# NVIDIA/audio-flamingo

Hardware: AMD Instinct MI355X
Metric: audio-sec/s + decoder tokens/s, AF3-7B bf16 train (higher is better)
Workload: dtype bf16; 1 GPU; AF3 (AF-Whisper 32L + Qwen2.5-7B 28L, MLP projector) bf16 train step fwd+bwd+AdamW, 30 s clips, S=1024; micro_batch_per_gpu=8, global_batch=8, seq_len=1024, parallelism=dp1, activation_checkpointing=False

## Files before the change

audio-flamingo_amd/csrc/gemm.hip:

```cpp
#include "gemm_common.h"
#include <vector>
#include <mutex>

namespace {

constexpr int BM = 128, BN = 128, BK = 64;
constexpr int ROWB = BK * 2;
constexpr int STAGE_BYTES = (BM + BN) * ROWB;
constexpr int NSTAGE = 2;

__global__ __launch_bounds__(256, 2) void gemm_nt_bf16_k128(GemmArgs p) {
    extern __shared__ __attribute__((aligned(16))) char smem[];
    const int tid = threadIdx.x;
    const int lane = tid & 63;
    const int wave = __builtin_amdgcn_readfirstlane(tid >> 6);
    const int wm = wave >> 1, wn = wave & 1;
    const int hi = lane >> 5, l31 = lane & 31;

    int tm, tn;
    gemm_tile_of_block(p, tm, tn);
    const int m0 = tm * BM, n0 = tn * BN;

    const bf16* a_src[4];
    const bf16* b_src[4];
// ... 140 lines not shown

__global__ __launch_bounds__(256) void gemm_splitk_reduce_kernel(GemmArgs p) {
    const int n4 = p.N >> 2;
    const int64_t total = (int64_t)p.M * n4;
    for (int64_t t = (int64_t)blockIdx.x * blockDim.x + threadIdx.x; t < total; t += (int64_t)gridDim.x * blockDim.x) {
        const int m = (int)(t / n4), n = (int)(t % n4) * 4;
        const float* src = p.ws + (int64_t)m * p.N + n;
        f32x4 acc = *(const f32x4*)src;
        for (int sp = 1; sp < p.splits; ++sp) {
            const f32x4 x = *(const f32x4*)(src + (int64_t)sp * p.M * p.N);
#pragma unroll
            for (int e = 0; e < 4; ++e) acc[e] += x[e];
        }
        float v[4] = {acc[0], acc[1], acc[2], acc[3]};
        gemm_epilogue_store4(p, m, n, v);
    }
}

struct ProfState {
    std::mutex mu;
    bool on = false;
    std::vector<hipEvent_t> pool;
    size_t used = 0;
    double flops = 0.0;
    int64_t launches = 0;
    struct Rec { int M, N, K, variant; };
    std::vector<Rec> recs;
};
ProfState g_prof;
int g_variant = 0;
[[maybe_unused]] int g_256_impl = 2;
int g_gm = 0;
int g_wide = 1;
int g_mfma = 0;

constexpr int mfma_shapes(int form) { return form == 0 ? AFK_MFMA_SHAPES_NT : form == 1 ? AFK_MFMA_SHAPES_NN : AFK_MFMA_SHAPES_TN; }
constexpr int AFK_MFMA_RULE_NT = 16, AFK_MFMA_RULE_NN = 32, AFK_MFMA_RULE_TN = 32;
int gemm_mfma_of(int form) {
    static const int env = [] {
        const char* e = getenv("AFK_GEMM_MFMA");
        return (e && e[0] >= '0' && e[0] <= '2' && !e[1]) ? e[0] - '0' : 0;
    }();
    const int sel = g_mfma ? g_mfma : env;
    if (sel == 1) return 32;
    if (sel == 2) return 16;
    return form == 0 ? AFK_MFMA_RULE_NT : form == 1 ? AFK_MFMA_RULE_NN : AFK_MFMA_RULE_TN;
}

hipEvent_t prof_next_event() {
    if (g_prof.used == g_prof.pool.size()) {
        hipEvent_t e;
        hipEventCreate(&e);
        g_prof.pool.push_back(e);
    }
    return g_prof.pool[g_prof.used++];
}

}

extern "C" int afk_gemm_set_variant(int v) {
    const int gm = (v >> 8) & 255, base = v & 15;
#ifdef AFK_PROBES
    AFK_REQUIRE(base >= 0 && base <= 14, "afk_gemm_set_variant: 14 = persistent tile loop with the next tile's prologue issued ahead of the epilogue stores (round-4 probe), 13 = 256x256 ping-pong as a persistent tile loop, 0 auto, 1 = 128x128, 2 = 256x256 8-wave ping-pong, 3 = 256x256 4-wave (4, 5: its timing probes), 6 = 256x256 8-wave free-running BK=64 (7, 8, 9: probes), 10 = 8-wave free-running BK=32 ring-10 (11: probe)");
#else
    AFK_REQUIRE(base >= 0 && base <= 2, "afk_gemm_set_variant: variant %d is a probe / rejected schedule; this libafk.so was built without -DAFK_PROBES (make PROBES=1)", base);
    AFK_REQUIRE((gm & 0xc0) == 0, "afk_gemm_set_variant: gm bits 6 / 7 are timing probes (wrong results); this libafk.so was built without -DAFK_PROBES");
#endif
    g_gm = gm;
    g_wide = (v & 16) ? 0 : 1;
    g_variant = base;
    return AFK_OK;
}

extern "C" int afk_gemm_set_mfma(int v) {
    AFK_REQUIRE(v >= 0 && v <= 2, "afk_gemm_set_mfma: %d (0 = dispatch rule, 1 = 32x32x16, 2 = 16x16x32)", v);
    constexpr int any = AFK_MFMA_SHAPES_NT | AFK_MFMA_SHAPES_NN | AFK_MFMA_SHAPES_TN;
    AFK_REQUIRE(v == 0 || (any >> (v - 1)) & 1, "afk_gemm_set_mfma: no 256x256 kernel of this libafk.so carries the %s shape; build with make PROBES=1",
                v == 1 ? "32x32x16" : "16x16x32");
    g_mfma = v;
    return AFK_OK;
}
extern "C" int afk_gemm_mfma_shapes(int form) { return form >= 0 && form <= 2 ? mfma_shapes(form) : 0; }

extern "C" int afk_prof_enable(int on) {
    std::lock_guard<std::mutex> lk(g_prof.mu);
    g_prof.on = on != 0;
    return AFK_OK;
}

extern "C" int afk_prof_reset(void) {
    std::lock_guard<std::mutex> lk(g_prof.mu);
    g_prof.used = 0;
    g_prof.flops = 0.0;
    g_prof.launches = 0;
    g_prof.recs.clear();
    return AFK_OK;
}

extern "C" int afk_prof_collect(double* total_ms, double* total_flops, int64_t* launches) {
    std::lock_guard<std::mutex> lk(g_prof.mu);
    double ms = 0.0;
// ... 26 lines not shown
    AFK_REQUIRE(M > 0 && N > 0 && K > 0, "afk_gemm_nt_bf16: bad shape %d %d %d", M, N, K);
    AFK_REQUIRE(!trans_a || trans_b, "afk_gemm_bf16: A^T with k-contiguous B is not implemented (NT, NN, TN are)");
    AFK_REQUIRE(trans_a || K % BK == 0, "afk_gemm_nt_bf16: K=%d must be a multiple of %d (pad the operand)", K, BK);
    AFK_REQUIRE(!trans_b || (N % 8 == 0 && N >= 8), "afk_gemm_bf16: N=%d must be a multiple of 8 for a reduction-major B", N);
    AFK_REQUIRE(!trans_a || (M % 8 == 0 && M >= 8), "afk_gemm_bf16: M=%d must be a multiple of 8 for a reduction-major A", M);
    AFK_REQUIRE(N % 4 == 0, "afk_gemm_nt_bf16: N=%d must be a multiple of 4", N);
    AFK_REQUIRE(lda % 8 == 0 && ldb % 8 == 0 && ldc % 4 == 0, "afk_gemm_nt_bf16: leading dims must keep 16-B (A,B) / 8-B (C) alignment");
    AFK_REQUIRE(!(flags & AFK_GEMM_BIAS) || bias, "afk_gemm_nt_bf16: BIAS flag without bias");
    AFK_REQUIRE(!(flags & AFK_GEMM_RESIDUAL) || (residual && ldr % 4 == 0), "afk_gemm_nt_bf16: RESIDUAL flag without residual");
    AFK_REQUIRE(!(flags & AFK_GEMM_SWIGLU_FWD) || (flags == AFK_GEMM_SWIGLU_FWD && !trans_a && !trans_b && preact_out && N % 256 == 0 && splits == 1 &&
                                                     ldc % 8 == 0 && (uintptr_t)C % 16 == 0 && (uintptr_t)preact_out % 16 == 0),
                "afk_gemm_nt_bf16: SWIGLU_FWD needs the NT form, preact_out, N = 2I with I %% 128 == 0 and no other flag");
    AFK_REQUIRE(!(flags & AFK_GEMM_SWIGLU_BWD) || (residual && ldr % 4 == 0 && ldc >= 2 * (int64_t)N && flags == AFK_GEMM_SWIGLU_BWD && splits == 1),
                "afk_gemm: SWIGLU_BWD needs the gate|up tensor as `residual`, a [M, 2N] output and no other epilogue flag");
    AFK_REQUIRE(((uintptr_t)A % 16 == 0) && ((uintptr_t)B % 16 == 0) && ((uintptr_t)C % 8 == 0), "afk_gemm_nt_bf16: misaligned pointer");
    GemmArgs p;
    p.A = (const bf16*)A;
    p.B = (const bf16*)B;
    p.C = C;
    p.C2 = preact_out;
    p.bias = (const bf16*)bias;
    p.R = (const bf16*)residual;
    p.lda = lda;
    p.ldb = ldb;
    p.ldc = ldc;
    p.ldr = ldr;
    p.M = M;
    p.N = N;
    p.K = K;
    p.flags = flags;
    p.res_mod = res_mod;
    p.alpha = alpha;
    p.gm = g_gm;
    p.splits = splits;
    p.ws = (float*)workspace;
    p.rope_cos = rope ? (const bf16*)rope->cos_t : nullptr;
    p.rope_sin = rope ? (const bf16*)rope->sin_t : nullptr;
    p.rope_pos = rope ? rope->pos : nullptr;
    p.rope_S = rope ? rope->S : 1;
    p.rope_cols = rope ? rope->cols : 0;
    const bool lanes_ok = rope && rope->cos_lanes && rope->sin_lanes && !rope->pos && rope->S % 32 == 0;
    p.rope_cos_lanes = lanes_ok ? (const bf16*)rope->cos_lanes : nullptr;
    p.rope_sin_lanes = lanes_ok ? (const bf16*)rope->sin_lanes : nullptr;
    {
        const bool f32 = (flags & AFK_GEMM_OUT_F32) != 0;
        bool w = N % 8 == 0 && ldc % 8 == 0 && (uintptr_t)C % (f32 ? 32 : 16) == 0;
        if (flags & AFK_GEMM_BIAS) w = w && (uintptr_t)bias % 16 == 0;
        if (flags & (AFK_GEMM_RESIDUAL | AFK_GEMM_SWIGLU_BWD)) w = w && ldr % 8 == 0 && (uintptr_t)residual % 16 == 0;
        if (preact_out) w = w && (uintptr_t)preact_out % 16 == 0;
        p.wide = w && g_wide ? 1 : 0;
    }
    const int64_t tiles256 = afk_cdiv(M, 256) * afk_cdiv(N, 256);
    const bool use256 = !gemv && (trans_b || (flags & AFK_GEMM_SWIGLU_FWD) || (splits == 1 && (g_variant >= 2 || (g_variant == 0 && tiles256 >= 192))));
    if (rope && (!use256 || !p.wide || trans_a || trans_b || splits != 1))
        return afk_set_error(AFK_ERR_UNSUPPORTED, "afk_gemm_nt_bf16_rope: needs the 256 x 256 NT kernel (>= 192 tiles) in its 16-byte epilogue form; use "
                                                  "afk_gemm_nt_bf16 + afk_rope_inplace for this shape");
#ifdef AFK_PROBES
    static const int env_impl = [] {
        const char* e = getenv("AFK_GEMM256");
        return (e && e[0] == 'p' && e[1] == 'e') ? 13 : (e && e[0] == 'p') ? 2 : (e && e[0] == 'w') ? 3 : (e && e[0] == 'f') ? 10 : 0;
    }();
    const int impl256 = (flags & (AFK_GEMM_SWIGLU_FWD | AFK_GEMM_ROPE)) ? 2 : g_variant >= 2 ? g_variant : (env_impl ? env_impl : g_256_impl);
    const bool w4 = use256 && !trans_b && impl256 >= 3 && impl256 <= 9;
    const bool f8 = use256 && !trans_b && impl256 >= 10 && impl256 <= 12;
    const bool persist = use256 && !trans_b && impl256 == 13;
    const bool persist_q = use256 && !trans_b && impl256 == 14;
// ... 130 lines not shown
```

audio-flamingo_amd/csrc/gemm256.hip:

```cpp
#include "gemm_common.h"

namespace {

constexpr int BM = 256, BN = 256, BK = 64;
constexpr int ROWB = 128;
constexpr int OP_BYTES = 256 * ROWB;
constexpr int BUF_BYTES = 2 * OP_BYTES;
constexpr int LDS_BYTES = 2 * BUF_BYTES;

#define AFK_VMCNT(n) asm volatile("s_waitcnt vmcnt(" #n ")" ::: "memory")
#define AFK_LGKMCNT0() asm volatile("s_waitcnt lgkmcnt(0)" ::: "memory")
#define AFK_BARRIER()                         \
    do {                                      \
        __builtin_amdgcn_sched_barrier(0);    \
        __builtin_amdgcn_s_barrier();         \
        __builtin_amdgcn_sched_barrier(0);    \
    } while (0)

template <int EPI, int MF>
__global__ __launch_bounds__(512, 1) void gemm_nt_bf16_k256(GemmArgs p) {
    extern __shared__ __attribute__((aligned(16))) char smem[];
    const int tid = threadIdx.x;
    const int lane = tid & 63;
    const int wave = __builtin_amdgcn_readfirstlane(tid >> 6);
    const int wm = wave >> 2, wn = wave & 3;
    const int hi = lane >> 5, l31 = lane & 31;

    int tm, tn;
    gemm_tile_of_block(p, tm, tn);
    const int m0 = tm * BM, n0 = tn * BN;

    const bf16* xsrc[6];
    int xdst[6];
    const bf16* ysrc[2];
    int ydst[2];
    {
        const int lrow = lane >> 3, pos = lane & 7;
#pragma unroll
        for (int j = 0; j < 6; ++j) {
            const int i = wave + 8 * j;
            const bool isB = i < 32;
            const int unit = isB ? i : ((i - 32) < 8 ? (i - 32) : (i - 32) + 8);
            const int rl = unit * 8 + lrow;
            const int chunk = pos ^ ((rl >> 1) & 7);
            if (isB) {
                const int r = (EPI == AFK_GEMM_SWIGLU_FWD) ? (rl < 128 ? tn * 128 + rl : (p.N >> 1) + tn * 128 + rl - 128) : min(n0 + rl, p.N - 1);
                xsrc[j] = p.B + (int64_t)r * p.ldb + chunk * 8;
            } else {
                const int r = min(m0 + rl, p.M - 1);
                xsrc[j] = p.A + (int64_t)r * p.lda + chunk * 8;
            }
            xdst[j] = (isB ? OP_BYTES : 0) + unit * 1024;
// ... 45 lines not shown
    AFK_BARRIER();
    if (wm == 1) AFK_BARRIER();

    bf16x8 bf[2][4], af[2][4];
    auto mfma_group = [&](auto acc0_, auto g_) {
        constexpr int ACC0 = decltype(acc0_)::value, g = decltype(g_)::value;
        if constexpr (MF == 32) {
#pragma unroll
            for (int i = 0; i < 2; ++i)
#pragma unroll
                for (int j = 0; j < 2; ++j) acc.mma(ACC0 + i, j, bf[j][g], af[i][g]);
        } else {
            constexpr int s = g >> 1, i = g & 1;
#pragma unroll
            for (int ih = 0; ih < 2; ++ih)
#pragma unroll
                for (int jt = 0; jt < 4; ++jt) acc.mma(2 * (ACC0 + i) + ih, jt, bf[jt >> 1][2 * (jt & 1) + s], af[i][2 * ih + s]);
        }
    };
    auto mfma_slot = [&](auto acc0_, auto q_) {
        constexpr int ACC0 = decltype(acc0_)::value, q = decltype(q_)::value;
        if constexpr (MF == 32) {
            constexpr int s = q >> 1, i = q & 1;
            acc.mma(ACC0 + i, 0, bf[0][s], af[i][s]);
            acc.mma(ACC0 + i, 1, bf[1][s], af[i][s]);
        } else {
            constexpr int s = q >> 2, i = (q >> 1) & 1, ih = q & 1;
#pragma unroll
            for (int jt = 0; jt < 4; ++jt) acc.mma(2 * (ACC0 + i) + ih, jt, bf[jt >> 1][2 * (jt & 1) + s], af[i][2 * ih + s]);
        }
    };
    using afk_c2 = std::integral_constant<int, 2>;
#define AFK_MFMA4(ACC0, g) mfma_group(std::integral_constant<int, ACC0>{}, std::integral_constant<int, g>{})
    for (int t = 0; t < T; ++t) {
        const char* buf = smem + (t & 1) * BUF_BYTES;
        const int t1 = min(t + 1, T - 1), t2 = min(t + 2, T - 1);
        const int e1 = (t + 1) & 1, e2 = t & 1;
        const int64_t oy = (int64_t)t1 * BK, ox = (int64_t)t2 * BK;
        char* by = smem + e1 * BUF_BYTES;
        char* bx = smem + e2 * BUF_BYTES;
#pragma unroll
        for (int j = 0; j < 2; ++j)
#pragma unroll
            for (int s = 0; s < 4; ++s) bf[j][s] = *(const bf16x8*)(buf + b_row0 + j * 32 * ROWB + koffb[s]);
#pragma unroll
        for (int i = 0; i < 2; ++i)
#pragma unroll
            for (int s = 0; s < 4; ++s) af[i][s] = *(const bf16x8*)(buf + a_row0 + i * 32 * ROWB + koffb[s]);
        AFK_LGKMCNT0();
        AFK_VMCNT(6);
        AFK_BARRIER();
        __builtin_amdgcn_s_setprio(1);
        AFK_MFMA4(0, 0);
        __builtin_amdgcn_sched_barrier(0);
        __builtin_amdgcn_global_load_lds((gbl_void*)(ysrc[0] + oy), (lds_void*)(by + ydst[0]), 16, 0, 0);
        __builtin_amdgcn_sched_barrier(0);
        AFK_MFMA4(0, 1);
        __builtin_amdgcn_sched_barrier(0);
        __builtin_amdgcn_global_load_lds((gbl_void*)(ysrc[1] + oy), (lds_void*)(by + ydst[1]), 16, 0, 0);
        __builtin_amdgcn_sched_barrier(0);
        AFK_MFMA4(0, 2);
        AFK_MFMA4(0, 3);
        __builtin_amdgcn_s_setprio(0);
        AFK_VMCNT(8);
        AFK_BARRIER();
#pragma unroll
        for (int i = 0; i < 2; ++i)
#pragma unroll
            for (int s = 0; s < 4; ++s) af[i][s] = *(const bf16x8*)(buf + a_row0 + (i + 2) * 32 * ROWB + koffb[s]);
        AFK_LGKMCNT0();
        AFK_VMCNT(2);
        AFK_BARRIER();
        __builtin_amdgcn_s_setprio(1);
        afk_static_for<8>([&](auto q_) {
            constexpr int piece = decltype(q_)::value;
            mfma_slot(afk_c2{}, q_);
            if constexpr (piece < 6) {
                __builtin_amdgcn_sched_barrier(0);
                __builtin_amdgcn_global_load_lds((gbl_void*)(xsrc[piece] + ox), (lds_void*)(bx + xdst[piece]), 16, 0, 0);
                __builtin_amdgcn_sched_barrier(0);
            }
        });
        __builtin_amdgcn_s_setprio(0);
        AFK_VMCNT(8);
        AFK_BARRIER();
    }
    AFK_VMCNT(0);
#undef AFK_MFMA4
    if (wm == 0) AFK_BARRIER();

    if constexpr (EPI == AFK_GEMM_SWIGLU_FWD) {
        typedef __attribute__((ext_vector_type(8))) __bf16 b8;
        const int I = p.N >> 1;
        const bool up = wn >= 2;
        const int feat0 = tn * 128 + (wn & 1) * 64;
        char* xch = smem + (wm * 2 + (wn & 1)) * 16384 + lane * 16;
        b8 pc[16];
#pragma unroll
        for (int i = 0; i < 4; ++i)
#pragma unroll
            for (int j = 0; j < 2; ++j)
#pragma unroll
                for (int t = 0; t < 2; ++t) {
                    const f32x16 blk = acc.block(i, j);
                    b8 o;
#pragma unroll
                    for (int e = 0; e < 4; ++e) {
                        float v0, v1;
                        gemm_lane_swap<MF>(blk[8 * t + e], blk[8 * t + 4 + e], v0, v1);
                        o[e] = (bf16)(v0 * p.alpha);
                        o[4 + e] = (bf16)(v1 * p.alpha);
                    }
                    pc[(i * 2 + j) * 2 + t] = o;
                }
        if (up) {
#pragma unroll
            for (int q = 0; q < 16; ++q) *(b8*)(xch + q * 1024) = pc[q];
        }
        __syncthreads();
#pragma unroll
        for (int i = 0; i < 4; ++i) {
            const int m = m0 + wm * 128 + i * 32 + l31;
// ... 70 lines not shown
                    const int cl = wn * 64 + j * 32 + 16 * t + 8 * hi;
                    b8 o = pc[q];
                    if (rot) {
                        const int d = cl & 127;
                        const b8 other = *(const b8*)(theirs + q * 1024);
                        const b8 c = lanes ? *(const b8*)(p.rope_cos_lanes + lbase + (d >> 3) * 256) : *(const b8*)(p.rope_cos + pr * 128 + d);
                        const b8 sn = lanes ? *(const b8*)(p.rope_sin_lanes + lbase + (d >> 3) * 256) : *(const b8*)(p.rope_sin + pr * 128 + d);
                        const float sg = (wn & 1) ? 1.f : -1.f;
#pragma unroll
                        for (int e = 0; e < 8; ++e)
                            o[e] = (bf16)(rbf_strict((float)pc[q][e] * (float)c[e]) + rbf_strict(sg * (float)other[e] * (float)sn[e]));
                    }
                    if (m < p.M) *(b8*)((bf16*)p.C + (int64_t)m * p.ldc + n0 + cl) = o;
                }
        }
        return;
    }
    if (AFK_GM_NOEPI(p)) return;
#pragma unroll
    for (int i = 0; i < 4; ++i)
#pragma unroll
        for (int j = 0; j < 2; ++j) gemm_store_block32<EPI, MF>(p, m0 + wm * 128 + i * 32, n0 + wn * 64 + j * 32, lane, acc.block(i, j));
}

}

#define AFK_EPI_LIST(X) X(0) X(AFK_GEMM_BIAS) X(AFK_GEMM_RESIDUAL) X(AFK_GEMM_BIAS | AFK_GEMM_RESIDUAL) X(AFK_GEMM_BIAS | AFK_GEMM_GELU) \
    X(AFK_GEMM_BIAS | AFK_GEMM_GELU | AFK_GEMM_RESIDUAL) X(AFK_GEMM_ACCUM) X(AFK_GEMM_SWIGLU_FWD) X(AFK_GEMM_SWIGLU_BWD) X(AFK_GEMM_ROPE) X(AFK_GEMM_ROPE | AFK_GEMM_BIAS) X(-1)

template <int MF>
static int launch_gemm256(const GemmArgs& p, hipStream_t st) {
    static bool attr_set = false;
    if (!attr_set) {
#define AFK_SET(F)                                                                                                                           \
    if (hipFuncSetAttribute((const void*)gemm_nt_bf16_k256<(F), MF>, hipFuncAttributeMaxDynamicSharedMemorySize, LDS_BYTES) != hipSuccess) \
        return afk_set_error(AFK_ERR_LAUNCH, "gemm256: cannot reserve %d bytes of LDS", LDS_BYTES);
        AFK_EPI_LIST(AFK_SET)
#undef AFK_SET
        attr_set = true;
    }
    const int64_t nwg = (int64_t)p.ntm * p.ntn;
    const int f = (p.wide && p.splits <= 1) ? p.flags : -1;
    switch (f) {
#define AFK_CASE(F)                                                                                              \
    case (F):                                                                                                    \
        if ((F) == -1) afk_count(AFK_CNT_GEMM_GENERIC);                                                          \
        hipLaunchKernelGGL((gemm_nt_bf16_k256<(F), MF>), dim3((unsigned)nwg), dim3(512), LDS_BYTES, st, p);      \
        break;
        AFK_EPI_LIST(AFK_CASE)
#undef AFK_CASE
        default:
            afk_count(AFK_CNT_GEMM_GENERIC);
            hipLaunchKernelGGL((gemm_nt_bf16_k256<-1, MF>), dim3((unsigned)nwg), dim3(512), LDS_BYTES, st, p);
    }
    return AFK_OK;
}

int afk_launch_gemm256(const GemmArgs& p, int mf, hipStream_t st) {
    if constexpr ((AFK_MFMA_SHAPES_NT & 2) != 0)
        if (mf == 16) return launch_gemm256<16>(p, st);
    if constexpr ((AFK_MFMA_SHAPES_NT & 1) != 0)
        if (mf == 32) return launch_gemm256<32>(p, st);
    return afk_set_error(AFK_ERR_UNSUPPORTED, "gemm256: the %s MFMA shape of the NT kernel is built under make PROBES=1 only", mf == 16 ? "16x16x32" : "32x32x16");
}
```

audio-flamingo_amd/csrc/gemm256t.hip:

```cpp
#include "gemm_common.h"

namespace {

constexpr int BK = 64;
constexpr int OP_BYTES = 32768;
constexpr int BUF_BYTES = 2 * OP_BYTES;
constexpr int LDS_BYTES = 2 * BUF_BYTES;
constexpr int TROW = 512;

typedef __attribute__((address_space(3))) bf16x4 lds_bf16x4;

#define AFK_VMCNT(n) asm volatile("s_waitcnt vmcnt(" #n ")" ::: "memory")
#define AFK_LGKMCNT0() asm volatile("s_waitcnt lgkmcnt(0)" ::: "memory")
#define AFK_BARRIER()                         \
    do {                                      \
        __builtin_amdgcn_sched_barrier(0);    \
        __builtin_amdgcn_s_barrier();         \
        __builtin_amdgcn_sched_barrier(0);    \
    } while (0)
#define AFK_DMA_PTR(SRCPTR, DSTPTR)                                                                       \
    do {                                                                                                  \
        __builtin_amdgcn_sched_barrier(0);                                                                \
        __builtin_amdgcn_global_load_lds((gbl_void*)(SRCPTR), (lds_void*)(DSTPTR), 16, 0, 0);             \
        __builtin_amdgcn_sched_barrier(0);                                                                \
    } while (0)

__device__ __forceinline__ int tswz(int r) { return ((r & 3) << 2) | ((r >> 2) & 3); }

template <int MF>
__device__ __forceinline__ int tr_off(int tile, int pc, int lane) {
    const int g = lane >> 4, i = lane & 15;
    const int chunk = MF == 16 ? 2 * tile + ((i & 3) >> 1) : 4 * tile + 2 * (g & 1) + ((i & 3) >> 1);
    const int r = (MF == 16 ? 8 * g : 8 * (g >> 1)) + (i >> 2) + 4 * pc;
    return r * TROW + ((chunk ^ tswz(r)) << 4) + 8 * (i & 1);
}
template <int MF, int S>
__device__ __forceinline__ bf16x8 tr_frag(uint32_t buf, int off0, int off1) {
    return afk_lds_tr_frag<S * (48 - MF) * TROW>(buf + off0, buf + off1);
}

struct TSrc {
    const bf16* base;
    int krow;
};
__device__ __forceinline__ TSrc tsrc(const bf16* mat, int unit, int col0, int ncols, int lane) {
    const int krow = 2 * unit + (lane >> 5);
    const int pos = lane & 31;
    const int chunk = pos ^ tswz(krow);
    const int col = min(col0 + chunk * 8, ncols - 8);
    TSrc s;
    s.base = mat + col;
    s.krow = krow;
    return s;
}

template <bool AT, int EPI, int MF>
__global__ __launch_bounds__(512, 1) void gemm_xt_bf16_k256(GemmArgs p) {
    extern __shared__ __attribute__((aligned(16))) char smem[];
    const int tid = threadIdx.x;
    const int lane = tid & 63;
    const int wave = __builtin_amdgcn_readfirstlane(tid >> 6);
    const int wm = wave >> 2, wn = wave & 3;
    const int hi = lane >> 5, l31 = lane & 31;

    int tm, tn;
    gemm_tile_of_block(p, tm, tn);
    const int m0 = tm * 256, n0 = tn * 256;
    int KL = p.K;
    const bf16* Abase = p.A;
    const bf16* Bbase = p.B;
    if (p.splits > 1) {
        const int tall = (p.K + BK - 1) / BK;
        const int t0 = (int)((int64_t)tall * blockIdx.y / p.splits), t1 = (int)((int64_t)tall * (blockIdx.y + 1) / p.splits);
        const int kbeg = t0 * BK;
        KL = min(p.K, t1 * BK) - kbeg;
        Abase += AT ? (int64_t)kbeg * p.lda : (int64_t)kbeg;
        Bbase += (int64_t)kbeg * p.ldb;
    }
    const int T = (KL + BK - 1) / BK;
    constexpr int NX = AT ? 4 : 6, NY = AT ? 4 : 2;

    const bf16* an_src[NX + NY];
    TSrc tr_src[NX + NY];
    int64_t tr_ld[NX + NY];
    int dst[NX + NY];
#pragma unroll
    for (int j = 0; j < NX + NY; ++j) {
        const bool isx = j < NX;
        const int jj = isx ? j : j - NX;
// ... 44 lines not shown
        return an_src[j] + (int64_t)t * BK;
    };
    auto issue = [&](int j, int t_src, int parity) { AFK_DMA_PTR(src_of(j, t_src), smem + parity * BUF_BYTES + dst[j]); };

    constexpr int NH = MF == 16 ? 2 : 1;
    int tob[2][NH][2], toa[4][NH][2];
#pragma unroll
    for (int j = 0; j < 2; ++j)
#pragma unroll
        for (int h = 0; h < NH; ++h)
#pragma unroll
            for (int pc = 0; pc < 2; ++pc) tob[j][h][pc] = OP_BYTES + tr_off<MF>((wn * 2 + j) * NH + h, pc, lane);
#pragma unroll
    for (int i = 0; i < 4; ++i)
#pragma unroll
        for (int h = 0; h < NH; ++h)
#pragma unroll
            for (int pc = 0; pc < 2; ++pc) toa[i][h][pc] = AT ? tr_off<MF>((wm * 4 + i) * NH + h, pc, lane) : 0;
    auto tr_read = [&](uint32_t lbuf, const int (&to)[NH][2], auto x_, auto ks0_) {
        constexpr int x = decltype(x_)::value, ks0 = decltype(ks0_)::value;
        if constexpr (MF == 32) return tr_frag<MF, ks0 + x>(lbuf, to[0][0], to[0][1]);
        else if constexpr (AT) return tr_frag<MF, ks0>(lbuf, to[x][0], to[x][1]);
        else return tr_frag<MF, (x & 1)>(lbuf, to[x >> 1][0], to[x >> 1][1]);
    };
    int koffb[4];
#pragma unroll
    for (int x = 0; x < 4; ++x) koffb[x] = gemm_frag_rowoff<MF>(x) * 128 + gemm_frag_koff<MF>(x, lane);
    const int a_row0 = (wm * 128 + gemm_frag_row<MF>(lane)) * 128;

#pragma unroll
    for (int j = 0; j < NX; ++j) issue(j, 0, 0);
#pragma unroll
    for (int j = 0; j < NY; ++j) issue(NX + j, 0, 0);
    {
        const int t1 = min(1, T - 1);
#pragma unroll
        for (int j = 0; j < NX; ++j) issue(j, t1, 1);
    }
    if (AT) AFK_VMCNT(8); else AFK_VMCNT(8);
    AFK_BARRIER();
    if (wm == 1) AFK_BARRIER();

    bf16x8 bf[2][4], af[AT ? 4 : 2][AT ? 2 : 4];
    const uint32_t lds0 = afk_lds_addr(smem);
    for (int t = 0; t < T; ++t) {
        const char* buf = smem + (t & 1) * BUF_BYTES;
        const uint32_t lbuf = lds0 + (t & 1) * BUF_BYTES;
        const int t1 = min(t + 1, T - 1), t2 = min(t + 2, T - 1);
        const int e1 = (t + 1) & 1, e2 = t & 1;
        if constexpr (!AT) {
#pragma unroll
            for (int j = 0; j < 2; ++j)
                afk_static_for<4>([&](auto x_) { bf[j][decltype(x_)::value] = tr_read(lbuf, tob[j], x_, std::integral_constant<int, 0>{}); });
#pragma unroll
            for (int i = 0; i < 2; ++i)
#pragma unroll
                for (int s = 0; s < 4; ++s) af[i][s] = *(const bf16x8*)(buf + a_row0 + i * 32 * 128 + koffb[s]);
            AFK_LGKMCNT0();
            AFK_VMCNT(6);
            AFK_BARRIER();
            __builtin_amdgcn_s_setprio(1);
            afk_static_for<4>([&](auto g_) {
                constexpr int g = decltype(g_)::value;
                if constexpr (MF == 32) {
#pragma unroll
                    for (int i = 0; i < 2; ++i)
#pragma unroll
                        for (int j = 0; j < 2; ++j) acc.mma(i, j, bf[j][g], af[i][g]);
                } else {
                    constexpr int s = g >> 1, i = g & 1;
#pragma unroll
                    for (int ih = 0; ih < 2; ++ih)
#pragma unroll
                        for (int jt = 0; jt < 4; ++jt) acc.mma(2 * i + ih, jt, bf[jt >> 1][2 * (jt & 1) + s], af[i][2 * ih + s]);
                }
                if constexpr (g < 2) issue(NX + g, t1, e1);
            });
            __builtin_amdgcn_s_setprio(0);
            AFK_VMCNT(8);
            AFK_BARRIER();
#pragma unroll
            for (int i = 0; i < 2; ++i)
#pragma unroll
                for (int s = 0; s < 4; ++s) af[i][s] = *(const bf16x8*)(buf + a_row0 + (i + 2) * 32 * 128 + koffb[s]);
            AFK_LGKMCNT0();
            AFK_VMCNT(2);
            AFK_BARRIER();
            __builtin_amdgcn_s_setprio(1);
            afk_static_for<8>([&](auto q_) {
                constexpr int piece = decltype(q_)::value;
                if constexpr (MF == 32) {
                    constexpr int s = piece >> 1, i = piece & 1;
                    acc.mma(2 + i, 0, bf[0][s], af[i][s]);
                    acc.mma(2 + i, 1, bf[1][s], af[i][s]);
                } else {
                    constexpr int s = piece >> 2, i = (piece >> 1) & 1, ih = piece & 1;
#pragma unroll
                    for (int jt = 0; jt < 4; ++jt) acc.mma(2 * (2 + i) + ih, jt, bf[jt >> 1][2 * (jt & 1) + s], af[i][2 * ih + s]);
                }
                if constexpr (piece < 6) issue(piece, t2, e2);
            });
            __builtin_amdgcn_s_setprio(0);
            AFK_VMCNT(8);
            AFK_BARRIER();
        } else {
            const int kvalid = KL - t * BK;
#pragma unroll
            for (int ph = 0; ph < 2; ++ph) {
                afk_static_for<2>([&](auto x_) {
                    constexpr int x = decltype(x_)::value;
                    constexpr int KS = MF == 16 ? 1 : 2;
                    if (ph == 0) {
#pragma unroll
                        for (int j = 0; j < 2; ++j) bf[j][x] = tr_read(lbuf, tob[j], x_, std::integral_constant<int, 0>{});
#pragma unroll
                        for (int i = 0; i < 4; ++i) af[i][x] = tr_read(lbuf, toa[i], x_, std::integral_constant<int, 0>{});
                    } else {
#pragma unroll
                        for (int j = 0; j < 2; ++j) bf[j][x] = tr_read(lbuf, tob[j], x_, std::integral_constant<int, KS>{});
#pragma unroll
                        for (int i = 0; i < 4; ++i) af[i][x] = tr_read(lbuf, toa[i], x_, std::integral_constant<int, KS>{});
                    }
                });
                AFK_LGKMCNT0();
                if (RAG && kvalid < BK) {
#pragma unroll
                    for (int s = 0; s < 2; ++s)
#pragma unroll
                        for (int e = 0; e < 8; ++e) {
                            const bool dead = (MF == 16 ? 32 * ph + 8 * (lane >> 4) : 16 * (2 * ph + s) + 8 * hi) + e >= kvalid;
#pragma unroll
                            for (int i = 0; i < 4; ++i)
                                if (dead) af[i][s][e] = (bf16)0.f;
                        }
                }
                AFK_VMCNT(4);
                AFK_BARRIER();
                __builtin_amdgcn_s_setprio(1);
                afk_static_for<8>([&](auto q_) {
                    constexpr int piece = decltype(q_)::value;
                    if constexpr (MF == 32) {
                        constexpr int s = piece >> 2, i = piece & 3;
                        acc.mma(i, 0, bf[0][s], af[i][s]);
                        acc.mma(i, 1, bf[1][s], af[i][s]);
                    } else {
                        constexpr int i = piece >> 1, ih = piece & 1;
#pragma unroll
                        for (int jt = 0; jt < 4; ++jt) acc.mma(2 * i + ih, jt, bf[jt >> 1][jt & 1], af[i][ih]);
                    }
                    if constexpr ((piece & 1) == 0) {
                        if (ph == 0) issue(NX + (piece >> 1), t1, e1);
                        else issue(piece >> 1, t2, e2);
                    }
                });
                __builtin_amdgcn_s_setprio(0);
                AFK_VMCNT(8);
                AFK_BARRIER();
            }
        }
    }
    AFK_VMCNT(0);
    if (wm == 0) AFK_BARRIER();
  };
    if (ragged) pipeline(std::true_type{});
    else pipeline(std::false_type{});

#pragma unroll
    for (int i = 0; i < 4; ++i)
#pragma unroll
        for (int j = 0; j < 2; ++j) gemm_store_block32<EPI, MF>(p, m0 + wm * 128 + i * 32, n0 + wn * 64 + j * 32, lane, acc.block(i, j));
}

}

#define AFK_EPI_LIST(X) X(0) X(AFK_GEMM_ACCUM) X(-2) X(-1)

template <bool AT, int MF>
static int launch_gemm256t(const GemmArgs& p, hipStream_t st) {
    static bool attr_set = false;
    if (!attr_set) {
#define AFK_SET(F)                                                                                                                              \
    if (hipFuncSetAttribute((const void*)gemm_xt_bf16_k256<AT, (F), MF>, hipFuncAttributeMaxDynamicSharedMemorySize, LDS_BYTES) != hipSuccess) \
        return afk_set_error(AFK_ERR_LAUNCH, "gemm256t: cannot reserve %d bytes of LDS", LDS_BYTES);
        AFK_EPI_LIST(AFK_SET)
#undef AFK_SET
        attr_set = true;
    }
    const int64_t nwg = (int64_t)p.ntm * p.ntn;
    const unsigned ns = (unsigned)(p.splits > 1 ? p.splits : 1);
    const int f = p.splits > 1 ? -2 : (p.wide ? p.flags : -1);
    const dim3 grid((unsigned)nwg, ns);
    switch (f) {
#define AFK_CASE(F)                                                                                        \
    case (F):                                                                                              \
        if ((F) == -1) afk_count(AFK_CNT_GEMM_GENERIC);                                                    \
        hipLaunchKernelGGL((gemm_xt_bf16_k256<AT, (F), MF>), grid, dim3(512), LDS_BYTES, st, p);           \
        break;
        AFK_EPI_LIST(AFK_CASE)
#undef AFK_CASE
        default:
            afk_count(AFK_CNT_GEMM_GENERIC);
            hipLaunchKernelGGL((gemm_xt_bf16_k256<AT, -1, MF>), grid, dim3(512), LDS_BYTES, st, p);
    }
    return AFK_OK;
}

int afk_launch_gemm256t(const GemmArgs& p, int trans_a, int mf, hipStream_t st) {
    if (trans_a) {
        if constexpr ((AFK_MFMA_SHAPES_TN & 2) != 0)
            if (mf == 16) return launch_gemm256t<true, 16>(p, st);
        if constexpr ((AFK_MFMA_SHAPES_TN & 1) != 0)
            if (mf == 32) return launch_gemm256t<true, 32>(p, st);
    } else {
        if constexpr ((AFK_MFMA_SHAPES_NN & 2) != 0)
            if (mf == 16) return launch_gemm256t<false, 16>(p, st);
        if constexpr ((AFK_MFMA_SHAPES_NN & 1) != 0)
            if (mf == 32) return launch_gemm256t<false, 32>(p, st);
    }
    return afk_set_error(AFK_ERR_UNSUPPORTED, "gemm256t: the %s MFMA shape of the %s kernel is built under make PROBES=1 only", mf == 16 ? "16x16x32" : "32x32x16",
                         trans_a ? "TN" : "NN");
}
```

audio-flamingo_amd/csrc/gemm_common.h:

```cpp
#pragma once
#include "common.h"
#include "../../include/afk.h"

struct GemmArgs {
    const bf16* A;
    const bf16* B;
    void* C;
    void* C2;
    const bf16* bias;
    const bf16* R;
    int64_t lda, ldb, ldc, ldr;
    int M, N, K;
    int ntm, ntn;
    int flags;
    int res_mod;
    float alpha;
    int gm;
    int splits;
    float* ws;
    int wide;
    const bf16* rope_cos;
    const bf16* rope_sin;
    const int* rope_pos;
    int rope_S, rope_cols;
    const bf16* rope_cos_lanes;
    const bf16* rope_sin_lanes;
};

#ifdef AFK_PROBES
#define AFK_GM_NOEPI(p) (((p).gm & 0x40) != 0)
#define AFK_GM_RAW(p) (((p).gm & 0x80) != 0)
#else
#define AFK_GM_NOEPI(p) false
#define AFK_GM_RAW(p) false
#endif

typedef __attribute__((address_space(3))) void lds_void;
typedef const __attribute__((address_space(1))) void gbl_void;

__device__ __forceinline__ void gemm_tile_of(const GemmArgs& p, int bid, int nwg, int& tm, int& tn) {
    const int xcd = bid & 7, idx = bid >> 3, q = nwg >> 3, r = nwg & 7;
    const int swz = AFK_GM_RAW(p) ? bid : (xcd < r ? xcd * (q + 1) : r * (q + 1) + (xcd - r) * q) + idx;
    const int GM = (p.gm & 0x3f) > 0 ? (p.gm & 0x3f) : 4;
    const int per_group = GM * p.ntn;
    const int g = swz / per_group, rem = swz - g * per_group;
    const int first_m = g * GM;
    const int gsz = min(p.ntm - first_m, GM);
    tm = first_m + rem % gsz;
    tn = rem / gsz;
}
__device__ __forceinline__ void gemm_tile_of_block(const GemmArgs& p, int& tm, int& tn) { gemm_tile_of(p, blockIdx.x, gridDim.x, tm, tn); }

template <int W, int F = -1>
__device__ __forceinline__ void gemm_epilogue_store(const GemmArgs& p, int m, int n, float* v) {
    typedef __attribute__((ext_vector_type(W))) __bf16 bvec;
    typedef __attribute__((ext_vector_type(W))) float fvec;
    const int flags = F >= 0 ? F : p.flags;
#pragma unroll
    for (int e = 0; e < W; ++e) v[e] *= p.alpha;
    if (flags & AFK_GEMM_BIAS) {
        const bvec bv = *(const bvec*)(p.bias + n);
#pragma unroll
        for (int e = 0; e < W; ++e) v[e] += (float)bv[e];
    }
    if (flags & AFK_GEMM_GELU) {
#pragma unroll
        for (int e = 0; e < W; ++e) v[e] = rbf(v[e]);
// ... 161 lines not shown
#pragma unroll
        for (int t = 0; t < 2; ++t) {
            float v[8];
#pragma unroll
            for (int e = 0; e < 4; ++e) gemm_lane_swap<MF>(b[8 * t + e], b[8 * t + 4 + e], v[e], v[4 + e]);
            const int n = nb + 16 * t + 8 * (lane >> 5);
            if (m < p.M && n < p.N) gemm_epilogue_store<8, F>(p, m, n, v);
        }
        return;
    }
#pragma unroll
    for (int t = 0; t < 2; ++t)
#pragma unroll
        for (int h = 0; h < 2; ++h) {
            int row, col;
            gemm_quad_pos<MF>(lane, t, h, row, col);
            const int m = mb + row, n = nb + col;
            if (m >= p.M || n >= p.N) continue;
            float v[4] = {b[8 * t + 4 * h], b[8 * t + 4 * h + 1], b[8 * t + 4 * h + 2], b[8 * t + 4 * h + 3]};
            gemm_epilogue_store<4, F>(p, m, n, v);
        }
}

#ifdef AFK_PROBES
#define AFK_MFMA_SHAPES_NT 3
#define AFK_MFMA_SHAPES_NN 3
#define AFK_MFMA_SHAPES_TN 3
#else
#define AFK_MFMA_SHAPES_NT 2
#define AFK_MFMA_SHAPES_NN 1
#define AFK_MFMA_SHAPES_TN 1
#endif

int afk_launch_gemm256(const GemmArgs& p, int mf, hipStream_t st);
int afk_launch_gemm256p(const GemmArgs& p, hipStream_t st);
int afk_launch_gemm256q(const GemmArgs& p, hipStream_t st);
int afk_launch_gemm256f8(const GemmArgs& p, int mode, hipStream_t st);
int afk_launch_gemm256w4(const GemmArgs& p, int mode, hipStream_t st);
int afk_launch_gemm256t(const GemmArgs& p, int trans_a, int mf, hipStream_t st);
```

Baseline: 629.7 audio-s/s.

## Peel K-loop tail in 256x256 GEMMs and prefetch SwiGLU-bwd operands

The 256x256 NT and TN GEMM kernels now peel the last two K-tiles instead of clamping the prefetch index. This drops the redundant global-to-LDS reloads of the final tile and lets the tail wait on exact vmcnt values. The NN kernel keeps the clamped loop by default, and A/B variant bits select either arm. The NT kernel also gains a dedicated SwiGLU-backward epilogue that issues the gate/up operand loads before the final barrier and interleaves them with the stores, hiding their latency at the cost of more registers and more template instantiations.

Result: no change. 633.8 audio-s/s, median of 6 (+0.7%).

```diff
diff --git a/audio-flamingo_amd/csrc/gemm.hip b/audio-flamingo_amd/csrc/gemm.hip
--- a/audio-flamingo_amd/csrc/gemm.hip
+++ b/audio-flamingo_amd/csrc/gemm.hip
@@ -196,6 +196,7 @@
 [[maybe_unused]] int g_256_impl = 2;
 int g_gm = 0;
 int g_wide = 1;
+int g_tail = 0;
 int g_mfma = 0;
 
 constexpr int mfma_shapes(int form) { return form == 0 ? AFK_MFMA_SHAPES_NT : form == 1 ? AFK_MFMA_SHAPES_NN : AFK_MFMA_SHAPES_TN; }
@@ -229,8 +230,11 @@
 #else
     AFK_REQUIRE(base >= 0 && base <= 2, "afk_gemm_set_variant: variant %d is a probe / rejected schedule; this libafk.so was built without -DAFK_PROBES (make PROBES=1)", base);
     AFK_REQUIRE((gm & 0xc0) == 0, "afk_gemm_set_variant: gm bits 6 / 7 are timing probes (wrong results); this libafk.so was built without -DAFK_PROBES");
+    AFK_REQUIRE((v & 96) == 0, "afk_gemm_set_variant: bits 5 / 6 (clamped / peeled K-loop tail) are A/B arms; this libafk.so was built without -DAFK_PROBES (make PROBES=1)");
 #endif
     g_gm = gm;
+    AFK_REQUIRE((v & 96) != 96, "afk_gemm_set_variant: bits 5 and 6 exclude each other");
+    g_tail = (v & 32) ? 1 : (v & 64) ? 2 : 0;
     g_wide = (v & 16) ? 0 : 1;
     g_variant = base;
     return AFK_OK;
@@ -323,6 +327,7 @@
     p.res_mod = res_mod;
     p.alpha = alpha;
     p.gm = g_gm;
+    p.clamped_tail = g_tail ? (g_tail == 1) : (trans_b ? (trans_a ? AFK_TAIL_CLAMPED_TN : AFK_TAIL_CLAMPED_NN) : AFK_TAIL_CLAMPED_NT);
     p.splits = splits;
     p.ws = (float*)workspace;
     p.rope_cos = rope ? (const bf16*)rope->cos_t : nullptr;
diff --git a/audio-flamingo_amd/csrc/gemm256.hip b/audio-flamingo_amd/csrc/gemm256.hip
--- a/audio-flamingo_amd/csrc/gemm256.hip
+++ b/audio-flamingo_amd/csrc/gemm256.hip
@@ -17,7 +17,18 @@
         __builtin_amdgcn_sched_barrier(0);    \
     } while (0)
 
-template <int EPI, int MF>
+__device__ __forceinline__ bf16x8 afk_gload16(const bf16* ptr) {
+    bf16x8 v;
+    asm volatile("global_load_dwordx4 %0, %1, off" : "=v"(v) : "v"(ptr) : "memory");
+    return v;
+}
+template <int N>
+__device__ __forceinline__ void afk_vmcnt_tie(bf16x8& a, bf16x8& b) {
+    static_assert(N >= 0 && N <= 63, "vmcnt is a 6-bit counter");
+    asm volatile("s_waitcnt vmcnt(%2)" : "+v"(a), "+v"(b) : "n"(N) : "memory");
+}
+
+template <int EPI, int MF, bool CLAMPED = false>
 __global__ __launch_bounds__(512, 1) void gemm_nt_bf16_k256(GemmArgs p) {
     extern __shared__ __attribute__((aligned(16))) char smem[];
     const int tid = threadIdx.x;
@@ -129,11 +140,12 @@
     };
     using afk_c2 = std::integral_constant<int, 2>;
 #define AFK_MFMA4(ACC0, g) mfma_group(std::integral_constant<int, ACC0>{}, std::integral_constant<int, g>{})
-    for (int t = 0; t < T; ++t) {
+    auto tile = [&](const int t, const int ty, const int tx, auto iy_, auto ix_) __attribute__((always_inline)) {
+        constexpr bool IY = decltype(iy_)::value, IX = decltype(ix_)::value;
+        static_assert(IY || !IX, "X(t+2) without Y(t+1) is no tile of the pipeline");
         const char* buf = smem + (t & 1) * BUF_BYTES;
-        const int t1 = min(t + 1, T - 1), t2 = min(t + 2, T - 1);
         const int e1 = (t + 1) & 1, e2 = t & 1;
-        const int64_t oy = (int64_t)t1 * BK, ox = (int64_t)t2 * BK;
+        const int64_t oy = (int64_t)ty * BK, ox = (int64_t)tx * BK;
         char* by = smem + e1 * BUF_BYTES;
         char* bx = smem + e2 * BUF_BYTES;
 #pragma unroll
@@ -145,46 +157,106 @@
 #pragma unroll
             for (int s = 0; s < 4; ++s) af[i][s] = *(const bf16x8*)(buf + a_row0 + i * 32 * ROWB + koffb[s]);
         AFK_LGKMCNT0();
-        AFK_VMCNT(6);
+        if constexpr (IY) AFK_VMCNT(6); else AFK_VMCNT(0);
         AFK_BARRIER();
         __builtin_amdgcn_s_setprio(1);
         AFK_MFMA4(0, 0);
-        __builtin_amdgcn_sched_barrier(0);
-        __builtin_amdgcn_global_load_lds((gbl_void*)(ysrc[0] + oy), (lds_void*)(by + ydst[0]), 16, 0, 0);
-        __builtin_amdgcn_sched_barrier(0);
+        if constexpr (IY) {
+            __builtin_amdgcn_sched_barrier(0);
+            __builtin_amdgcn_global_load_lds((gbl_void*)(ysrc[0] + oy), (lds_void*)(by + ydst[0]), 16, 0, 0);
+            __builtin_amdgcn_sched_barrier(0);
+        }
         AFK_MFMA4(0, 1);
-        __builtin_amdgcn_sched_barrier(0);
-        __builtin_amdgcn_global_load_lds((gbl_void*)(ysrc[1] + oy), (lds_void*)(by + ydst[1]), 16, 0, 0);
-        __builtin_amdgcn_sched_barrier(0);
+        if constexpr (IY) {
+            __builtin_amdgcn_sched_barrier(0);
+            __builtin_amdgcn_global_load_lds((gbl_void*)(ysrc[1] + oy), (lds_void*)(by + ydst[1]), 16, 0, 0);
+            __builtin_amdgcn_sched_barrier(0);
+        }
         AFK_MFMA4(0, 2);
         AFK_MFMA4(0, 3);
         __builtin_amdgcn_s_setprio(0);
-        AFK_VMCNT(8);
+        if constexpr (IY) AFK_VMCNT(8); else AFK_VMCNT(0);
         AFK_BARRIER();
 #pragma unroll
         for (int i = 0; i < 2; ++i)
 #pragma unroll
             for (int s = 0; s < 4; ++s) af[i][s] = *(const bf16x8*)(buf + a_row0 + (i + 2) * 32 * ROWB + koffb[s]);
         AFK_LGKMCNT0();
-        AFK_VMCNT(2);
+        if constexpr (IY) AFK_VMCNT(2); else AFK_VMCNT(0);
         AFK_BARRIER();
         __builtin_amdgcn_s_setprio(1);
         afk_static_for<8>([&](auto q_) {
             constexpr int piece = decltype(q_)::value;
             mfma_slot(afk_c2{}, q_);
-            if constexpr (piece < 6) {
+            if constexpr (IX && piece < 6) {
                 __builtin_amdgcn_sched_barrier(0);
                 __builtin_amdgcn_global_load_lds((gbl_void*)(xsrc[piece] + ox), (lds_void*)(bx + xdst[piece]), 16, 0, 0);
                 __builtin_amdgcn_sched_barrier(0);
             }
         });
         __builtin_amdgcn_s_setprio(0);
-        AFK_VMCNT(8);
+        if constexpr (IX) AFK_VMCNT(8); else if constexpr (IY) AFK_VMCNT(2); else AFK_VMCNT(0);
         AFK_BARRIER();
+    };
+    if constexpr (CLAMPED) {
+        for (int t = 0; t < T; ++t) tile(t, min(t + 1, T - 1), min(t + 2, T - 1), std::true_type{}, std::true_type{});
+    } else {
+        for (int t = 0; t < T - 2; ++t) tile(t, t + 1, t + 2, std::true_type{}, std::true_type{});
+        if (T > 1) tile(T - 2, T - 1, 0, std::true_type{}, std::false_type{});
+        tile(T - 1, 0, 0, std::false_type{}, std::false_type{});
     }
     AFK_VMCNT(0);
 #undef AFK_MFMA4
+    typedef bf16x8 sb8;
+    [[maybe_unused]] sb8 sgv[16], suv[16];
+    [[maybe_unused]] auto swiglu_bwd_load = [&](auto q_) __attribute__((always_inline)) {
+        constexpr int q = decltype(q_)::value, i = q >> 2, j = (q >> 1) & 1, t = q & 1;
+        const int m = min(m0 + wm * 128 + i * 32 + l31, p.M - 1);
+        const int n = min(n0 + wn * 64 + j * 32 + 16 * t + 8 * hi, p.N - 8);
+        const bf16* r = p.R + (int64_t)m * p.ldr + n;
+        sgv[q] = afk_gload16(r);
+        suv[q] = afk_gload16(r + p.N);
+    };
+    if constexpr (EPI == AFK_GEMM_SWIGLU_BWD) {
+        afk_static_for<8>([&](auto q_) { swiglu_bwd_load(q_); });
+        __builtin_amdgcn_sched_barrier(0);
+    }
     if (wm == 0) AFK_BARRIER();
+
+    if constexpr (EPI == AFK_GEMM_SWIGLU_BWD) {
+        afk_static_for<16>([&](auto q_) {
+            constexpr int q = decltype(q_)::value, i = q >> 2, j = (q >> 1) & 1, t = q & 1;
+            const int m = m0 + wm * 128 + i * 32 + l31;
+            const int n = n0 + wn * 64 + j * 32 + 16 * t + 8 * hi;
+            const f32x16 blk = acc.block(i, j);
+            float v[8];
+#pragma unroll
+            for (int e = 0; e < 4; ++e) gemm_lane_swap<MF>(blk[8 * t + e], blk[8 * t + 4 + e], v[e], v[4 + e]);
+#pragma unroll
+            for (int e = 0; e < 8; ++e) v[e] *= p.alpha;
+            afk_vmcnt_tie<(q < 8 ? 14 : 2 * (15 - q))>(sgv[q], suv[q]);
+            const sb8 gv = sgv[q], uv = suv[q];
+            sb8 og, ou;
+#pragma unroll
+            for (int e = 0; e < 8; ++e) {
+                const float gf = (float)gv[e], uf = (float)uv[e], df = rbf(v[e]);
+                const float s = sigmoid_f(gf);
+                og[e] = (bf16)(df * uf * (s * (1.f + gf * (1.f - s))));
+                ou[e] = (bf16)(df * (gf * s));
+            }
+            if (m < p.M && n < p.N) {
+                bf16* cp = (bf16*)p.C + (int64_t)m * p.ldc + n;
+                *(sb8*)cp = og;
+                *(sb8*)(cp + p.N) = ou;
+            }
+            if constexpr (q < 8) {
+                __builtin_amdgcn_sched_barrier(0);
+                swiglu_bwd_load(std::integral_constant<int, q + 8>{});
+                __builtin_amdgcn_sched_barrier(0);
+            }
+        });
+        return;
+    }
 
     if constexpr (EPI == AFK_GEMM_SWIGLU_FWD) {
         typedef __attribute__((ext_vector_type(8))) __bf16 b8;
@@ -321,27 +393,41 @@
 static int launch_gemm256(const GemmArgs& p, hipStream_t st) {
     static bool attr_set = false;
     if (!attr_set) {
-#define AFK_SET(F)                                                                                                                           \
-    if (hipFuncSetAttribute((const void*)gemm_nt_bf16_k256<(F), MF>, hipFuncAttributeMaxDynamicSharedMemorySize, LDS_BYTES) != hipSuccess) \
+#define AFK_SET_(F, CL)                                                                                                                          \
+    if (hipFuncSetAttribute((const void*)gemm_nt_bf16_k256<(F), MF, CL>, hipFuncAttributeMaxDynamicSharedMemorySize, LDS_BYTES) != hipSuccess) \
         return afk_set_error(AFK_ERR_LAUNCH, "gemm256: cannot reserve %d bytes of LDS", LDS_BYTES);
+#ifdef AFK_PROBES
+#define AFK_SET(F) AFK_SET_(F, false) AFK_SET_(F, true)
+#else
+#define AFK_SET(F) AFK_SET_(F, AFK_TAIL_CLAMPED_NT != 0)
+#endif
         AFK_EPI_LIST(AFK_SET)
 #undef AFK_SET
+#undef AFK_SET_
         attr_set = true;
     }
     const int64_t nwg = (int64_t)p.ntm * p.ntn;
     const int f = (p.wide && p.splits <= 1) ? p.flags : -1;
     switch (f) {
-#define AFK_CASE(F)                                                                                              \
-    case (F):                                                                                                    \
-        if ((F) == -1) afk_count(AFK_CNT_GEMM_GENERIC);                                                          \
-        hipLaunchKernelGGL((gemm_nt_bf16_k256<(F), MF>), dim3((unsigned)nwg), dim3(512), LDS_BYTES, st, p);      \
+#ifdef AFK_PROBES
+#define AFK_LAUNCH(F)                                                                                                             \
+    if (AFK_GM_CLAMPED_TAIL(p, false)) hipLaunchKernelGGL((gemm_nt_bf16_k256<(F), MF, true>), dim3((unsigned)nwg), dim3(512), LDS_BYTES, st, p); \
+    else hipLaunchKernelGGL((gemm_nt_bf16_k256<(F), MF, false>), dim3((unsigned)nwg), dim3(512), LDS_BYTES, st, p)
+#else
+#define AFK_LAUNCH(F) hipLaunchKernelGGL((gemm_nt_bf16_k256<(F), MF, AFK_TAIL_CLAMPED_NT != 0>), dim3((unsigned)nwg), dim3(512), LDS_BYTES, st, p)
+#endif
+#define AFK_CASE(F)                                                 \
+    case (F):                                                       \
+        if ((F) == -1) afk_count(AFK_CNT_GEMM_GENERIC);             \
+        AFK_LAUNCH(F);                                              \
         break;
         AFK_EPI_LIST(AFK_CASE)
 #undef AFK_CASE
         default:
             afk_count(AFK_CNT_GEMM_GENERIC);
-            hipLaunchKernelGGL((gemm_nt_bf16_k256<-1, MF>), dim3((unsigned)nwg), dim3(512), LDS_BYTES, st, p);
-    }
+            AFK_LAUNCH(-1);
+    }
+#undef AFK_LAUNCH
     return AFK_OK;
 }
 
diff --git a/audio-flamingo_amd/csrc/gemm256t.hip b/audio-flamingo_amd/csrc/gemm256t.hip
--- a/audio-flamingo_amd/csrc/gemm256t.hip
+++ b/audio-flamingo_amd/csrc/gemm256t.hip
@@ -54,7 +54,7 @@
     return s;
 }
 
-template <bool AT, int EPI, int MF>
+template <bool AT, int EPI, int MF, bool CLAMPED = false>
 __global__ __launch_bounds__(512, 1) void gemm_xt_bf16_k256(GemmArgs p) {
     extern __shared__ __attribute__((aligned(16))) char smem[];
     const int tid = threadIdx.x;
@@ -165,21 +165,26 @@
     for (int j = 0; j < NX; ++j) issue(j, 0, 0);
 #pragma unroll
     for (int j = 0; j < NY; ++j) issue(NX + j, 0, 0);
-    {
+    if (T > 1 || CLAMPED) {
         const int t1 = min(1, T - 1);
 #pragma unroll
         for (int j = 0; j < NX; ++j) issue(j, t1, 1);
-    }
-    if (AT) AFK_VMCNT(8); else AFK_VMCNT(8);
+        AFK_VMCNT(8);
+    } else if constexpr (AT) {
+        AFK_VMCNT(4);
+    } else {
+        AFK_VMCNT(2);
+    }
     AFK_BARRIER();
     if (wm == 1) AFK_BARRIER();
 
     bf16x8 bf[2][4], af[AT ? 4 : 2][AT ? 2 : 4];
     const uint32_t lds0 = afk_lds_addr(smem);
-    for (int t = 0; t < T; ++t) {
+    auto tile = [&](const int t, const int t1, const int t2, auto iy_, auto ix_) __attribute__((always_inline)) {
+        constexpr bool IY = decltype(iy_)::value, IX = decltype(ix_)::value;
+        static_assert(IY || !IX, "X(t+2) without Y(t+1) is no tile of the pipeline");
         const char* buf = smem + (t & 1) * BUF_BYTES;
         const uint32_t lbuf = lds0 + (t & 1) * BUF_BYTES;
-        const int t1 = min(t + 1, T - 1), t2 = min(t + 2, T - 1);
         const int e1 = (t + 1) & 1, e2 = t & 1;
         if constexpr (!AT) {
 #pragma unroll
@@ -190,7 +195,7 @@
 #pragma unroll
                 for (int s = 0; s < 4; ++s) af[i][s] = *(const bf16x8*)(buf + a_row0 + i * 32 * 128 + koffb[s]);
             AFK_LGKMCNT0();
-            AFK_VMCNT(6);
+            if constexpr (IY) AFK_VMCNT(6); else AFK_VMCNT(0);
             AFK_BARRIER();
             __builtin_amdgcn_s_setprio(1);
             afk_static_for<4>([&](auto g_) {
@@ -207,17 +212,17 @@
 #pragma unroll
                         for (int jt = 0; jt < 4; ++jt) acc.mma(2 * i + ih, jt, bf[jt >> 1][2 * (jt & 1) + s], af[i][2 * ih + s]);
                 }
-                if constexpr (g < 2) issue(NX + g, t1, e1);
+                if constexpr (IY && g < 2) issue(NX + g, t1, e1);
             });
             __builtin_amdgcn_s_setprio(0);
-            AFK_VMCNT(8);
+            if constexpr (IY) AFK_VMCNT(8); else AFK_VMCNT(0);
             AFK_BARRIER();
 #pragma unroll
             for (int i = 0; i < 2; ++i)
 #pragma unroll
                 for (int s = 0; s < 4; ++s) af[i][s] = *(const bf16x8*)(buf + a_row0 + (i + 2) * 32 * 128 + koffb[s]);
             AFK_LGKMCNT0();
-            AFK_VMCNT(2);
+            if constexpr (IY) AFK_VMCNT(2); else AFK_VMCNT(0);
             AFK_BARRIER();
             __builtin_amdgcn_s_setprio(1);
             afk_static_for<8>([&](auto q_) {
@@ -231,10 +236,10 @@
 #pragma unroll
                     for (int jt = 0; jt < 4; ++jt) acc.mma(2 * (2 + i) + ih, jt, bf[jt >> 1][2 * (jt & 1) + s], af[i][2 * ih + s]);
                 }
-                if constexpr (piece < 6) issue(piece, t2, e2);
+                if constexpr (IX && piece < 6) issue(piece, t2, e2);
             });
             __builtin_amdgcn_s_setprio(0);
-            AFK_VMCNT(8);
+            if constexpr (IX) AFK_VMCNT(8); else if constexpr (IY) AFK_VMCNT(2); else AFK_VMCNT(0);
             AFK_BARRIER();
         } else {
             const int kvalid = KL - t * BK;
@@ -267,7 +272,7 @@
                                 if (dead) af[i][s][e] = (bf16)0.f;
                         }
                 }
-                AFK_VMCNT(4);
+                if constexpr (IY) AFK_VMCNT(4); else AFK_VMCNT(0);
                 AFK_BARRIER();
                 __builtin_amdgcn_s_setprio(1);
                 afk_static_for<8>([&](auto q_) {
@@ -282,21 +287,38 @@
                         for (int jt = 0; jt < 4; ++jt) acc.mma(2 * i + ih, jt, bf[jt >> 1][jt & 1], af[i][ih]);
                     }
                     if constexpr ((piece & 1) == 0) {
-                        if (ph == 0) issue(NX + (piece >> 1), t1, e1);
-                        else issue(piece >> 1, t2, e2);
+                        if (ph == 0) {
+                            if constexpr (IY) issue(NX + (piece >> 1), t1, e1);
+                        } else {
+                            if constexpr (IX) issue(piece >> 1, t2, e2);
+                        }
                     }
                 });
                 __builtin_amdgcn_s_setprio(0);
-                AFK_VMCNT(8);
+                if (ph == 0) {
+                    if constexpr (IY) AFK_VMCNT(8); else AFK_VMCNT(0);
+                } else {
+                    if constexpr (IX) AFK_VMCNT(8); else if constexpr (IY) AFK_VMCNT(4); else AFK_VMCNT(0);
+                }
                 AFK_BARRIER();
             }
         }
+    };
+    if constexpr (CLAMPED) {
+        for (int t = 0; t < T; ++t) tile(t, min(t + 1, T - 1), min(t + 2, T - 1), std::true_type{}, std::true_type{});
+    } else {
+        for (int t = 0; t < T - 2; ++t) tile(t, t + 1, t + 2, std::true_type{}, std::true_type{});
+        if (T > 1) tile(T - 2, T - 1, 0, std::true_type{}, std::false_type{});
+        tile(T - 1, 0, 0, std::false_type{}, std::false_type{});
     }
     AFK_VMCNT(0);
     if (wm == 0) AFK_BARRIER();
   };
-    if (ragged) pipeline(std::true_type{});
-    else pipeline(std::false_type{});
+    if (AT && ragged) {
+        if constexpr (AT) pipeline(std::true_type{});
+    } else {
+        pipeline(std::false_type{});
+    }
 
 #pragma unroll
     for (int i = 0; i < 4; ++i)
@@ -310,13 +332,20 @@
 
 template <bool AT, int MF>
 static int launch_gemm256t(const GemmArgs& p, hipStream_t st) {
+    constexpr bool RULE = (AT ? AFK_TAIL_CLAMPED_TN : AFK_TAIL_CLAMPED_NN) != 0;
     static bool attr_set = false;
     if (!attr_set) {
-#define AFK_SET(F)                                                                                                                              \
-    if (hipFuncSetAttribute((const void*)gemm_xt_bf16_k256<AT, (F), MF>, hipFuncAttributeMaxDynamicSharedMemorySize, LDS_BYTES) != hipSuccess) \
+#define AFK_SET_(F, CL)                                                                                                                             \
+    if (hipFuncSetAttribute((const void*)gemm_xt_bf16_k256<AT, (F), MF, CL>, hipFuncAttributeMaxDynamicSharedMemorySize, LDS_BYTES) != hipSuccess) \
         return afk_set_error(AFK_ERR_LAUNCH, "gemm256t: cannot reserve %d bytes of LDS", LDS_BYTES);
+#ifdef AFK_PROBES
+#define AFK_SET(F) AFK_SET_(F, false) AFK_SET_(F, true)
+#else
+#define AFK_SET(F) AFK_SET_(F, RULE)
+#endif
         AFK_EPI_LIST(AFK_SET)
 #undef AFK_SET
+#undef AFK_SET_
         attr_set = true;
     }
     const int64_t nwg = (int64_t)p.ntm * p.ntn;
@@ -324,17 +353,25 @@
     const int f = p.splits > 1 ? -2 : (p.wide ? p.flags : -1);
     const dim3 grid((unsigned)nwg, ns);
     switch (f) {
-#define AFK_CASE(F)                                                                                        \
-    case (F):                                                                                              \
-        if ((F) == -1) afk_count(AFK_CNT_GEMM_GENERIC);                                                    \
-        hipLaunchKernelGGL((gemm_xt_bf16_k256<AT, (F), MF>), grid, dim3(512), LDS_BYTES, st, p);           \
+#ifdef AFK_PROBES
+#define AFK_LAUNCH(F)                                                                                                  \
+    if (AFK_GM_CLAMPED_TAIL(p, RULE)) hipLaunchKernelGGL((gemm_xt_bf16_k256<AT, (F), MF, true>), grid, dim3(512), LDS_BYTES, st, p); \
+    else hipLaunchKernelGGL((gemm_xt_bf16_k256<AT, (F), MF, false>), grid, dim3(512), LDS_BYTES, st, p)
+#else
+#define AFK_LAUNCH(F) hipLaunchKernelGGL((gemm_xt_bf16_k256<AT, (F), MF, RULE>), grid, dim3(512), LDS_BYTES, st, p)
+#endif
+#define AFK_CASE(F)                                                 \
+    case (F):                                                       \
+        if ((F) == -1) afk_count(AFK_CNT_GEMM_GENERIC);             \
+        AFK_LAUNCH(F);                                              \
         break;
         AFK_EPI_LIST(AFK_CASE)
 #undef AFK_CASE
         default:
             afk_count(AFK_CNT_GEMM_GENERIC);
-            hipLaunchKernelGGL((gemm_xt_bf16_k256<AT, -1, MF>), grid, dim3(512), LDS_BYTES, st, p);
-    }
+            AFK_LAUNCH(-1);
+    }
+#undef AFK_LAUNCH
     return AFK_OK;
 }
 
diff --git a/audio-flamingo_amd/csrc/gemm_common.h b/audio-flamingo_amd/csrc/gemm_common.h
--- a/audio-flamingo_amd/csrc/gemm_common.h
+++ b/audio-flamingo_amd/csrc/gemm_common.h
@@ -25,14 +25,17 @@
     int rope_S, rope_cols;
     const bf16* rope_cos_lanes;
     const bf16* rope_sin_lanes;
+    int clamped_tail;
 };
 
 #ifdef AFK_PROBES
 #define AFK_GM_NOEPI(p) (((p).gm & 0x40) != 0)
 #define AFK_GM_RAW(p) (((p).gm & 0x80) != 0)
+#define AFK_GM_CLAMPED_TAIL(p, RULE) ((p).clamped_tail != 0)
 #else
 #define AFK_GM_NOEPI(p) false
 #define AFK_GM_RAW(p) false
+#define AFK_GM_CLAMPED_TAIL(p, RULE) (RULE)
 #endif
 
 typedef __attribute__((address_space(3))) void lds_void;
@@ -260,6 +263,10 @@
 #define AFK_MFMA_SHAPES_TN 1
 #endif
 
+#define AFK_TAIL_CLAMPED_NT 0
+#define AFK_TAIL_CLAMPED_NN 1
+#define AFK_TAIL_CLAMPED_TN 0
+
 int afk_launch_gemm256(const GemmArgs& p, int mf, hipStream_t st);
 int afk_launch_gemm256p(const GemmArgs& p, hipStream_t st);
 int afk_launch_gemm256q(const GemmArgs& p, hipStream_t st);
```
